# relife957/FastApriori

Hardware: AMD Instinct MI355X
Metric: itemsets/sec (mining wall-clock), T10I4D100M min_sup=0.001 (higher is better)
Workload: dtype int32/uint64-bitmap (exact integer counts); 1 GPU; model=T10I4D100M, global_batch=100000000, parallelism=dp1, n_itemsets=33139, min_count=100000

## Files before the change

### csrc/hip/regroup.hip

```cpp
#include "fa_hip.h"
#include "../host/fa_dl.h"
#include "../host/fa_regroup.h"

namespace fa {

constexpr int kRgThreads = 1024;
constexpr int kRgW = kRgThreads / 64;

struct RgLv {
  const int32_t* P;
  const int32_t* cnt;
  const int64_t* off;
  const int32_t* rows;
  char* scr;
  int64_t n, C, base;
  int64_t m;
};
struct RgArgs {
  RgLv lv[kDlMaxL];
  int32_t* perm;
  long long* stats;
};

__host__ __device__ inline int64_t rg_scratch_ints(int64_t n, int64_t C, int64_t m) {
  return ((C * (m + 5) + n) + 1) & ~(int64_t)1;
}
__host__ __device__ inline int64_t rg_scratch_bytes(int64_t n, int64_t C, int64_t m) {
  return (4 * rg_scratch_ints(n, C, m) + 8 * (n + 1) + 255) & ~(int64_t)255;
}

__device__ __forceinline__ int rg_find(const int32_t* __restrict__ P, int n, int m, const int32_t* __restrict__ s,
                                       int j) {
  int lo = 0, hi = n;
  while (lo < hi) {
    const int mid = (lo + hi) >> 1;
    const int r = cmp_skip(P + (int64_t)mid * m, s, m + 1, j);
    if (r == 0) return mid;
    if (r < 0) lo = mid + 1; else hi = mid;
  }
  return -1;
}

__global__ __launch_bounds__(kRgThreads) void k_dl_regroup(const RgArgs A) {
  extern __shared__ int rg_lds[];
  __shared__ int sh[2 * kRgW];
  __shared__ int fired;
  const RgLv& V = A.lv[blockIdx.x];
  const int tid = threadIdx.x;
  const int64_t C = V.C, base = V.base;
  if (V.n > kRgMaxRows) {
    for (int64_t c = tid; c < C; c += kRgThreads) A.perm[base + c] = (int32_t)(base + c);
    int pp = 0;
    for (int64_t i = tid; i < V.n; i += kRgThreads) pp += (V.cnt[i] + 7) >> 3;
    pp = wg_sum<kRgW>(pp, sh);
    if (tid == 0) {
      long long* s = A.stats + 4 * blockIdx.x;
      s[0] = s[1] = pp; s[2] = 0; s[3] = 1;
    }
    return;
  }
  const int n = (int)V.n, m = (int)V.m, k = m + 1;
  int32_t* const par = reinterpret_cast<int32_t*>(V.scr);
  int32_t* const asg = par + C * k;
  int32_t* const cho = asg + C;
  int32_t* const tmp = cho + C;
  int32_t* const cnt_out = tmp + C;
  int32_t* const ex_out = cnt_out + n;
  int64_t* const off_out = reinterpret_cast<int64_t*>(V.scr + 4 * rg_scratch_ints(n, C, m));
  int* u = rg_lds;
  int* u2 = rg_lds + n;
  int* const v = rg_lds + 2 * n;
  for (int i = tid; i < 3 * n; i += kRgThreads) rg_lds[i] = 0;
  if (tid == 0) fired = 0;
  __syncthreads();
  for (int64_t c = tid; c < C; c += kRgThreads) {
    const int32_t* s = V.rows + c * k;
    int lo = 0, hi = n;
    while (lo < hi) {
      const int mid = (lo + hi) >> 1;
      if (V.off[mid] <= c) lo = mid + 1; else hi = mid;
    }
    for (int j = 0; j < m; ++j) par[c * k + j] = rg_find(V.P, n, m, s, j);
    par[c * k + m] = lo - 1;
    asg[c] = -1;
    for (int j = 0; j < k; ++j) {
      const int p = par[c * k + j];
      if (p >= 0) atomicAdd(&u[p], 1);
    }
  }
  __syncthreads();
  int rounds = 0;
  for (int t = 0; t < kRgNThr; ++t) {
    const int thr = rg_thr(t);
    for (;;) {
      ++rounds;
      for (int64_t c = tid; c < C; c += kRgThreads) {
        if (asg[c] >= 0) continue;
        int best = -1, bp = -1;
        for (int j = k - 1; j >= 0; --j) {
          const int p = par[c * k + j];
          if (p < 0) continue;
          const int uu = u[p];
          if (uu >= thr && uu > best) { best = uu; bp = p; }
        }
        cho[c] = bp;
        if (bp >= 0) atomicAdd(&v[bp], 1);
      }
      __syncthreads();
      for (int64_t c = tid; c < C; c += kRgThreads) {
        if (asg[c] >= 0) continue;
        const int bp = cho[c];
        if (bp >= 0 && v[bp] >= thr) {
          asg[c] = bp;
          fired = 1;
          continue;
        }
        for (int j = 0; j < k; ++j) {
          const int p = par[c * k + j];
          if (p >= 0) atomicAdd(&u2[p], 1);
        }
      }
      __syncthreads();
      const int f = fired;
      __syncthreads();
      if (tid == 0) fired = 0;
      if (f) { int* x = u; u = u2; u2 = x; }
      for (int i = tid; i < n; i += kRgThreads) { u2[i] = 0; v[i] = 0; }
      __syncthreads();
      if (!f) break;
    }
  }
  for (int64_t c = tid; c < C; c += kRgThreads) atomicAdd(&v[asg[c]], 1);
  __syncthreads();
  int pc[2] = {0, 0}, tot[2];
  for (int i = tid; i < n; i += kRgThreads) {
    pc[0] += (v[i] + 7) >> 3;
    pc[1] += (V.cnt[i] + 7) >> 3;
  }
  wg_sum<kRgW>(pc, sh, tot);
  const bool keep = tot[0] >= tot[1];
  __syncthreads();
  if (keep) {
    for (int i = tid; i < n; i += kRgThreads) v[i] = 0;
    __syncthreads();
    for (int64_t c = tid; c < C; c += kRgThreads) {
      asg[c] = par[c * k + m];
      atomicAdd(&v[asg[c]], 1);
    }
    __syncthreads();
  }
  for (int i = tid; i < n; i += kRgThreads) cnt_out[i] = v[i];
  wg_scan_chunks<kRgW>(
      (int64_t)n, (int64_t)0, sh, [&](int64_t i) { return v[i]; },
      [&](int64_t i, int64_t before, int) { off_out[i] = before; });
  if (tid == 0) off_out[n] = C;
  for (int64_t c = tid; c < C; c += kRgThreads) {
    const int p = asg[c];
    tmp[off_out[p] + atomicAdd(&u2[p], 1)] = (int32_t)c;
  }
  __syncthreads();
  for (int64_t c = tid; c < C; c += kRgThreads) {
    const int p = asg[c];
    const int64_t o = off_out[p];
    const int a = v[p];
    int r = 0;
    for (int q = 0; q < a; ++q) r += tmp[o + q] < (int32_t)c ? 1 : 0;
    int j = m;
    if (!keep)
      for (j = k - 1; j > 0 && par[c * k + j] != p; --j) {}
    ex_out[o + r] = V.rows[c * k + j];
    A.perm[base + o + r] = (int32_t)(base + c);
  }
  if (tid == 0) {
    long long* s = A.stats + 4 * blockIdx.x;
    s[0] = tot[1]; s[1] = tot[0]; s[2] = rounds; s[3] = keep ? 1 : 0;
  }
}

__global__ __launch_bounds__(256) void k_dl_unpermute(const uint32_t* __restrict__ in, const int32_t* __restrict__ perm,
                                                      int64_t C, uint32_t* __restrict__ out) {
  const int64_t e = (int64_t)blockIdx.x * 256 + threadIdx.x;
  if (e < C) out[perm[e]] = in[e];
}

static inline int64_t rg_al(int64_t b) { return (b + 255) & ~(int64_t)255; }

static bool rg_eligible(const DlDesc* desc, int L) {
  if (L < 1 || L > kDlMaxL) return false;
  for (int l = 0; l < L; ++l)
    if (desc[l].m < 1 || desc[l].m > kDlInline || desc[l].n < 1 || desc[l].C < 1 || desc[l].C > INT32_MAX / 64)
      return false;
  return true;
}

}

using namespace fa;

FA_API int64_t fa_hip_dl_regroup_need(const DlDesc* desc, int L) {
  if (!rg_eligible(desc, L)) return 0;
  int64_t C = 0, b = 0;
  for (int l = 0; l < L; ++l) {
    C += desc[l].C;
    if (desc[l].n <= kRgMaxRows) b += rg_scratch_bytes(desc[l].n, desc[l].C, desc[l].m);
  }
  return rg_al(4 * C) + b;
}

FA_API int fa_hip_dl_regroup(const DlDesc* desc, int L, void* scratch, int64_t bytes, DlDesc* out, long long* stats,
                             hipStream_t st) {
  const int64_t need = fa_hip_dl_regroup_need(desc, L);
  if (need == 0 || scratch == nullptr || stats == nullptr || bytes < need) return 1;
  int64_t C = 0;
  for (int l = 0; l < L; ++l) C += desc[l].C;
  RgArgs A{};
  char* w = static_cast<char*>(scratch);
  A.perm = reinterpret_cast<int32_t*>(w);
  w += rg_al(4 * C);
  A.stats = stats;
  int64_t n_max = 1;
  for (int l = 0; l < L; ++l) {
    const DlDesc& d = desc[l];
    RgLv& V = A.lv[l];
    V.P = reinterpret_cast<const int32_t*>((intptr_t)d.P);
    V.cnt = reinterpret_cast<const int32_t*>((intptr_t)d.cnt);
    V.off = reinterpret_cast<const int64_t*>((intptr_t)d.off);
    V.rows = reinterpret_cast<const int32_t*>((intptr_t)d.rows);
    V.n = d.n; V.C = d.C; V.base = d.base; V.m = d.m;
    V.scr = w;
    out[l] = d;
    if (d.n > kRgMaxRows) continue;
    n_max = std::max(n_max, d.n);
    int32_t* cnt_out = reinterpret_cast<int32_t*>(w) + d.C * (d.m + 1) + 3 * d.C;
    out[l].cnt = (int64_t)(intptr_t)cnt_out;
    out[l].off = (int64_t)(intptr_t)(w + 4 * rg_scratch_ints(d.n, d.C, d.m));
    w += rg_scratch_bytes(d.n, d.C, d.m);
  }
  const size_t lds = 3 * sizeof(int) * (size_t)n_max;
  static bool lds_set = false;
  if (!lds_set) {
    const hipError_t e = hipFuncSetAttribute((const void*)k_dl_regroup, hipFuncAttributeMaxDynamicSharedMemorySize,
                                             (int)(3 * sizeof(int) * kRgMaxRows));
    if (e != hipSuccess) return (int)e;
    lds_set = true;
  }
  hipLaunchKernelGGL(k_dl_regroup, dim3((unsigned)L), dim3(kRgThreads), lds, st, A);
  FA_LAUNCH_RET();
}

FA_API int fa_hip_dl_unpermute(const uint32_t* in, const int32_t* perm, int64_t C, uint32_t* out, hipStream_t st) {
  if (C < 1) return 1;
  hipLaunchKernelGGL(k_dl_unpermute, dim3((unsigned)((C + 255) / 256)), dim3(256), 0, st, in, perm, C, out);
  FA_LAUNCH_RET();
}
```

### csrc/host/fa_regroup.h

```cpp
#pragma once
#include <stdint.h>

namespace fa {

constexpr int kRgNThr = 6;
constexpr int rg_thr(int t) { return t == 0 ? 8 : t == 1 ? 6 : t == 2 ? 4 : t == 3 ? 3 : t == 4 ? 2 : 1; }
constexpr int kRgMaxRows = 12288;
constexpr int kRgStats = 224;
static_assert(kRgStats + 4 * 32 <= 512, "the statistics end before the control block's bitset");

inline int rg_cmp_skip(const int32_t* a, const int32_t* s, int k, int p) {
  for (int i = 0, j = 0; i < k - 1; ++i, ++j) {
    if (j == p) ++j;
    const int32_t x = a[i], y = s[j];
    if (x != y) return x < y ? -1 : 1;
  }
  return 0;
}

}
```

### fastapriori_amd/ops/_native.py

```python
from __future__ import annotations

import ctypes as C
import os
import threading

from . import build as _build

_lock = threading.Lock()
_host = None
_hip = None

i32, i64, u64, dbl = C.c_int32, C.c_int64, C.c_uint64, C.c_double
vp, cp = C.c_void_p, C.c_char_p
I64P = C.POINTER(C.c_int64)
IP = C.POINTER(C.c_int)

_HOST_SIGS = {
    "fa_parse_file": (vp, [cp, i64, i64, C.c_int, C.c_int, IP]),
    "fa_parse_buffer": (vp, [cp, i64, C.c_int, C.c_int]),
    "fa_file_size": (i64, [cp]),
    "fa_next_line_start": (i64, [cp, i64, i64]),
    "fa_chunk_scan": (None, [vp, i64, vp]),
    "fa_txndb_info": (None, [vp, vp]),
    "fa_txndb_export": (None, [vp, vp, vp, vp, C.c_int]),
# ... 25 lines not shown
    "fa_slab_tail_cut": (C.c_int, [vp, C.c_int, i64, dbl, dbl]),
    "fa_trim_estimate": (None, [vp, i64, dbl, C.c_int, C.POINTER(dbl), C.POINTER(dbl)]),
    "fa_dl_layout": (cp, [C.c_int, I64P]),
    "fa_limits": (cp, [C.c_int, I64P]),
    "fa_query_limits": (cp, [C.c_int, I64P]),
    "fa_query_lds_bytes": (i64, [i64, i64, i64]),
    "fa_query_width": (C.c_int, [i64, i64, i64]),
    "fa_query_plan": (vp, [vp, vp, vp, i64, i64, i64, i64]),
    "fa_query_plan_info": (None, [vp, vp]),
    "fa_query_plan_export": (None, [vp, vp, vp, vp, vp, vp]),
    "fa_query_plan_free": (None, [vp]),
    "fa_query_count_cpu": (C.c_int, [vp, vp, i64, vp, i64, vp, i64, vp, vp, vp, vp, vp, i64, C.c_int]),
    "fa_f1_rank_numeric": (i64, [vp, i64, i64, vp, vp, vp]),
    "fa_rules_build": (vp, [vp, vp, vp, C.c_int, vp, C.c_int, vp]),
    "fa_rules_nante": (i64, [vp]),
    "fa_rules_nstats": (i64, [vp]),
    "fa_rules_export": (None, [vp, vp, vp, vp, vp, vp]),
    "fa_rules_free": (None, [vp]),
    "fa_rule_measures_cpu": (vp, [vp, vp, vp, vp, C.c_int, i64, dbl, C.c_int, dbl, C.c_int, i64, vp, C.c_int, vp]),
    "fa_rule_measures_nante": (i64, [vp]),
    "fa_rule_measures_export": (None, [vp] * 12),
    "fa_rule_measures_free": (None, [vp]),
    "fa_write_rules": (C.c_int, [cp, cp] + [vp] * 12 + [i64, C.c_int]),
    "fa_recommend_cpu": (None, [vp, vp, vp, i64, i32, vp, vp, i64, vp, C.c_int]),
    "fa_recommend_topn_cpu": (None, [vp, vp, vp, i64, i32, vp, vp, i64, i32, vp, C.c_int]),
    "fa_holdout_rank_cpu": (None, [vp, vp, vp, i64, i32, vp, vp, vp, i64, i32, vp, C.c_int]),
    "fa_recommend_combined_cpu": (None, [vp, vp, vp, vp, i64, i32, vp, vp, i64, i32, vp, vp, C.c_int]),
    "fa_holdout_rank_combined_cpu": (None, [vp, vp, vp, vp, i64, i32, vp, vp, vp, i64, i32, vp, C.c_int]),
    "fa_combine_wave_bytes": (i64, [i64]),
    "fa_combine_waves": (C.c_int, [i64]),
    "fa_combine_lds_max": (i64, []),
    "fa_condense_cpu": (C.c_int, [vp, vp, vp, vp, C.c_int, vp, vp, C.c_int]),
    "fa_write_freq_itemsets": (C.c_int, [cp, vp, vp, i32, vp, vp, vp, C.c_int, C.c_int, C.c_int]),
    "fa_cpu_histogram": (None, [vp, i64, i64, vp, C.c_int]),
    "fa_build_probe_table": (None, [vp, i64, C.c_int, C.c_uint32, vp, vp]),
    "fa_cpu_txn_freq_count": (None, [vp, vp, i64, vp, vp, C.c_int]),
    "fa_cpu_compress": (None, [vp, vp, vp, vp, i64, vp, vp, C.c_int]),
    "fa_cpu_build_bitmaps": (None, [vp, vp, vp, i64, i64, vp, C.c_int]),
    "fa_cpu_row_hash": (None, [vp, vp, i64, vp, vp, C.c_int]),
    "fa_cpu_pair_gram": (None, [vp, i32, i64, i64, vp, vp, C.c_int]),
    "fa_cpu_pair_horizontal": (None, [vp, vp, i64, vp, i32, vp, C.c_int]),
    "fa_cpu_count_candidates": (None, [vp, i64, i64, vp, i32, vp, vp, i64, vp, vp, C.c_int]),
}

_HIP_SIGS = {
    "fa_hip_histogram": (C.c_int, [vp, i64, i32, vp, vp]),
    "fa_hip_f1_rank": (C.c_int, [vp, i32, i64, C.c_int, vp, vp, vp]),
    "fa_hip_debug_la_qsum": (C.c_int, [vp, vp]),
    "fa_hip_win_alive": (C.c_int, [vp, i64, vp, C.c_int, i64, C.c_int, vp, vp, vp]),
    "fa_hip_win_compact": (C.c_int, [vp, i64, vp, C.c_int, i64, vp, vp, vp, i64, vp]),
    "fa_hip_debug_slab_max_wg": (None, [C.c_int]),
    "fa_hip_pairs_compact": (C.c_int, [vp, i64, i32, i64, vp, vp, vp, vp, vp, vp]),
    "fa_hip_f1_sketch": (C.c_int, [vp, i64, vp, vp, vp]),
    "fa_hip_f1_exact": (C.c_int, [vp, i64, vp, C.c_int, vp, vp]),
    "fa_hip_txn_freq_count": (C.c_int, [vp, vp, i64, i64, vp, vp, vp]),
    "fa_hip_compress_regs": (C.c_int, [C.c_int, vp, vp, vp, vp, i64, vp, vp, vp, vp, vp]),
    "fa_hip_ag_gen": (C.c_int, [vp, i64, C.c_int, C.c_int, vp, i64, vp, i64, vp, vp]),
    "fa_hip_ag_chain": (C.c_int, [vp, i64, C.c_int, C.c_int, vp, i64, vp, i64, C.c_int, dbl, i64, i64, vp, vp,
                                  C.c_int, dbl]),
    "fa_hip_ag_build": (C.c_int, [vp, i64, C.c_int, vp, C.c_uint32, C.c_int, vp, vp]),
    "fa_hip_ag_rows": (C.c_int, [vp, i64, C.c_int, vp, C.c_uint32, C.c_int, vp, vp, vp, vp, C.c_int, vp]),
    "fa_hip_cmp_agg": (C.c_int, [vp, vp, vp, i64, vp, vp, vp, C.c_int, vp]),
    "fa_hip_cmp_scan": (C.c_int, [vp, vp, i64, C.c_int, vp, vp, vp, vp, vp]),
    "fa_hip_cmp_emit": (C.c_int, [vp, vp, vp, i64, vp, vp, vp, vp, vp, vp, vp, vp, C.c_int, vp, vp, i64, vp, vp,
                                  vp]),
    "fa_hip_lr_rows": (C.c_int, [vp, vp, vp, i64, vp, C.c_int, vp, i64, vp]),
    "fa_hip_compress_regs_bc": (C.c_int, [vp, vp, vp, vp, i64, vp, vp, vp, vp, vp, i64, C.c_int, vp]),
    "fa_hip_block_counts_rows": (C.c_int, [vp, vp, vp, i64, vp, i64, C.c_int, vp, vp]),
    "fa_hip_block_bsum": (C.c_int, [vp, i64, i64, C.c_int, vp, vp]),
    "fa_hip_compress_staged": (C.c_int, [vp, vp, vp, i64, vp, vp, vp, vp, vp]),
    "fa_hip_compress_staged64": (C.c_int, [vp, vp, vp, i64, vp, vp, vp, vp, C.c_int, vp]),
    "fa_hip_count_slab_rec_cls": (C.c_int, [vp, vp, vp, i64, vp, C.c_int, C.c_int, vp, vp, C.c_int, C.c_int, vp,
                                            vp, C.c_int, C.c_int, vp, i64, vp, vp, vp, C.c_int]),
    "fa_hip_dl_level0": (C.c_int, [vp, vp, i64, i64, C.c_int, C.c_int, vp, i64, vp, vp, i64, dbl, dbl, vp, C.c_int,
                                   vp]),
    "fa_hip_dl_more": (C.c_int, [C.c_int, vp, i64, i64, vp, vp, dbl, C.c_int, dbl, dbl, i64, vp, vp, vp, vp]),
    "fa_hip_dl_plan": (C.c_int, [vp, C.c_int, vp, C.c_int, vp, vp, i64, vp, i64, vp, i64, C.c_int, vp]),
    "fa_hip_set_lane_deal": (None, [C.c_int]),
    "fa_hip_set_dl_tail": (None, [dbl, C.c_int]),
    "fa_hip_set_piece_part": (C.c_int, [C.c_int, C.c_int]),
    "fa_hip_set_dl_regroup": (None, [C.c_int]),
    "fa_hip_dl_regroup_last": (None, [vp]),
    "fa_hip_dl_regroup_need": (i64, [vp, C.c_int]),
    "fa_hip_dl_regroup": (C.c_int, [vp, C.c_int, vp, i64, vp, vp, vp]),
    "fa_hip_dl_unpermute": (C.c_int, [vp, vp, i64, vp, vp]),
    "fa_hip_dl_gpre_need": (i64, [vp, C.c_int]),
    "fa_hip_dl_plan_window": (C.c_int, [vp, C.c_int, vp, C.c_int, vp, vp, i64, vp, i64, vp, i64, i64, i64, C.c_int,
                                        vp]),
    "fa_hip_dl_plan_window_bits": (C.c_int, [vp, C.c_int, vp, C.c_int, vp, vp, vp, i64, vp, i64, vp, i64, i64, i64,
                                             C.c_int, vp]),
    "fa_hip_dl_chunk_bits": (C.c_int, [vp, C.c_int, C.c_int, vp, vp]),
    "fa_hip_dl_threshold": (C.c_int, [vp, C.c_int, vp, i64, vp, vp, vp, vp, vp, vp, i64, vp]),
    "fa_hip_trim_scan_count": (C.c_int, [vp, vp, i64, vp, C.c_int, C.c_int, vp, vp, vp, vp, vp]),
    "fa_hip_trim_emit": (C.c_int, [vp, vp, vp, C.c_int, i64, vp, vp, vp, vp, vp, vp, vp, vp]),
    "fa_hip_compress_wave": (C.c_int, [vp, vp, vp, vp, i64, vp, vp, vp, C.c_int, vp, vp]),
    "fa_hip_compress_lds": (C.c_int, [vp, vp, vp, vp, i64, vp, vp, vp, vp, vp, vp]),
    "fa_hip_dedup_probe": (C.c_int, [vp, vp, vp, i64, vp, vp, vp]),
    "fa_hip_row_hash": (C.c_int, [vp, vp, i64, vp, vp, vp]),
    "fa_hip_build_bitmaps": (C.c_int, [vp, vp, vp, i64, i32, i64, C.c_int, C.c_int, vp, vp, vp, C.c_int, vp]),
    "fa_hip_block_counts": (C.c_int, [vp, vp, i64, i32, vp, vp, C.c_int, vp]),
    "fa_hip_block_scatter": (C.c_int, [vp, vp, i64, i32, vp, vp, vp, C.c_int, vp]),
    "fa_hip_pair_queue16": (C.c_int, [vp, vp, vp, i64, C.c_int, i64, vp, vp, C.c_int, vp]),
    "fa_hip_pair_blocked": (C.c_int, [vp, vp, vp, i64, vp, i32, vp, i64, vp]),
    "fa_hip_pair_gram_mfma": (C.c_int, [vp, i32, i64, i64, C.c_int, i64, vp, C.c_int, C.c_uint32, C.c_int, vp]),
    "fa_hip_pair_gram_popc": (C.c_int, [vp, i32, i64, i64, C.c_int, i64, vp, vp, C.c_int, vp]),
    "fa_hip_count_candidates": (C.c_int, [vp, i64, i64, vp, C.c_int, vp, vp, vp, C.c_int, vp, vp, vp]),
    "fa_hip_recommend": (C.c_int, [vp, vp, vp, i64, i32, vp, vp, i64, vp, vp]),
    "fa_hip_recommend_indexed": (C.c_int, [vp, vp, vp, vp, vp, i64, i32, vp, vp, i64, vp, vp]),
    "fa_hip_recommend_topn": (C.c_int, [vp, vp, vp, i64, i32, vp, vp, i64, i32, vp, vp]),
    "fa_hip_recommend_topn_indexed": (C.c_int, [vp, vp, vp, vp, vp, i64, i32, vp, vp, i64, i32, vp, vp]),
    "fa_hip_holdout_rank": (C.c_int, [vp, vp, vp, i64, i32, vp, vp, vp, i64, i32, vp, vp]),
    "fa_hip_holdout_rank_indexed": (C.c_int, [vp, vp, vp, vp, vp, i64, i32, vp, vp, vp, i64, i32, vp, vp]),
    "fa_hip_recommend_combined": (C.c_int, [vp, vp, vp, vp, vp, vp, i64, i32, vp, vp, i64, i32, vp, vp, vp]),
    "fa_hip_holdout_rank_combined": (C.c_int, [vp, vp, vp, vp, vp, vp, i64, i32, vp, vp, vp, i64, i32, vp, vp]),
    "fa_hip_parse_tiles": (i64, [i64]),
    "fa_hip_tparse_tiles": (i64, [i64, i64]),
    "fa_hip_tline_count": (C.c_int, [vp, i64, i64, vp, vp]),
    "fa_hip_tparse": (C.c_int, [vp, i64, i64, i64, C.c_int, i64, vp, vp, vp, vp, vp, vp, vp, vp, vp]),
    "fa_hip_scan_small": (C.c_int, [C.c_int, vp, i64, vp, vp, vp]),
    "fa_hip_tcompact": (C.c_int, [vp, vp, i64, C.c_int, vp, vp, vp, vp, vp, vp, vp, i64, i64, vp, C.c_int, vp, vp, vp]),
    "fa_hip_hist_reduce": (C.c_int, [vp, C.c_int, vp, vp]),
    "fa_hip_line_count": (C.c_int, [vp, i64, vp, vp]),
    "fa_hip_line_ends": (C.c_int, [vp, i64, vp, vp, vp]),
    "fa_hip_parse_lines_dict": (C.c_int, [vp, vp, i64, vp, vp, vp, vp, vp, vp, vp, vp, vp, i64, vp]),
    "fa_hip_slot_remap": (C.c_int, [vp, i64, vp, vp]),
    "fa_hip_dict_verify": (C.c_int, [vp, vp, i64, vp, vp, vp, vp, i64, vp]),
    "fa_hip_compact_lines": (C.c_int, [vp, vp, vp, vp, vp, vp, vp, i64, vp, vp, vp]),
    "fa_hip_rule_gen": (C.c_int, [vp, i64, C.c_int, vp, i64, vp, vp, vp, vp, vp, vp]),
    "fa_hip_rule_cut": (C.c_int, [vp, vp, i64, C.c_int, vp, vp, vp, vp]),
    "fa_hip_rule_emit": (C.c_int, [vp, vp, vp, vp, vp, i64, vp, vp]),
    "fa_hip_rule_measures": (C.c_int, [vp, vp, vp, vp, vp, vp, C.c_int, i64, dbl, C.c_int, dbl, C.c_int, vp, vp, vp,
                                       vp, vp]),
    "fa_hip_rule_measures_emit": (C.c_int, [vp, vp, vp, vp, vp, vp, C.c_int, i64, C.c_int, vp, vp, i64, vp, vp, vp,
                                            vp, vp, vp, vp, vp, vp]),
    "fa_hip_rule_measures_fin": (C.c_int, [vp, vp, vp, i64, i64, vp, vp, vp, vp, vp, vp]),
    "fa_hip_sup_mark": (C.c_int, [vp, vp, vp, vp, vp, vp, C.c_int, vp, vp, vp, vp]),
    "fa_hip_query_count": (C.c_int, [vp, vp, i64, vp, i64, vp, vp, i64, vp, vp, vp, vp, vp, i64, C.c_int, vp]),
}


def _declare(lib, sigs):
    for name, (res, args) in sigs.items():
        fn = getattr(lib, name)
        fn.restype = res
        fn.argtypes = args
    return lib


BUILD_IDS: dict = {}


def _check_id(kind: str, lib, path: str) -> None:
    fn = lib.fa_build_id
    fn.restype, fn.argtypes = cp, []
    got = fn().decode("ascii", "replace")
    have_src = bool(_build.hip_sources() if kind == "hip" else _build.host_sources())
    want = _build.source_id(kind) if have_src else None
    BUILD_IDS[kind] = (got, want, path)
    override = kind == "hip" and bool(os.environ.get("FA_HIP_LIB"))
    if want is not None and got != want and not override:
        raise RuntimeError(f"{path} was built from other sources (build id {got}, these sources {want}): "
                           "rebuild with `python -m fastapriori_amd.ops.build`")


def host():
    global _host
# ... 33 lines not shown
```

### fastapriori_amd/ops/primitives.py

```python
from __future__ import annotations

import ctypes as C
import ctypes
import functools
import os
import time
from dataclasses import dataclass

import numpy as np
import torch

from ..tuning import TUNING
from ..utils.env import num_threads
from . import _native
from .host import rule_measures_plan, rules_gap_level, rules_not_closed

_I32, _I64 = torch.int32, torch.int64
PAIR_CHUNK_ROWS = 1 << 18


def _p(t: torch.Tensor | None) -> int | None:
    return None if t is None else t.data_ptr()


# ... 1745 lines not shown
        self.rows_hint = 0

    def grow(self, nbytes: int) -> None:
        self.ws = torch.empty(int(nbytes * 1.25) + (1 << 20), dtype=torch.uint8, device=self.dev)

    def post_buffers(self, F1: int, c_cap: int, rows_cap: int, gpre_n: int = 0):
        part_n = 8 * ((rows_cap + 255) // 256 + 2)
        b = self.post_bufs
        if (b is None or b["F1"] < F1 or b["c_cap"] < c_cap or b["part"].numel() < part_n
                or b["gpre"].numel() < gpre_n):
            F1, c_cap = max(F1, b["F1"] if b else 0), max(c_cap, b["c_cap"] if b else 0)
            part_n = max(part_n, b["part"].numel() if b else 0)
            gpre_n = max(gpre_n, b["gpre"].numel() if b else 1)
            b = self.post_bufs = dict(F1=F1, c_cap=c_cap,
                                      item_map=torch.empty(max(F1, 1), dtype=_I32, device=self.dev),
                                      rec=torch.empty(12 * c_cap + 12, dtype=_I32, device=self.dev),
                                      part=torch.empty(part_n, dtype=_I32, device=self.dev),
                                      out=torch.empty(c_cap, dtype=_I32, device=self.dev),
                                      gpre=torch.empty(max(gpre_n, 1), dtype=_I32, device=self.dev))
        return b


_DL_STATE: dict = {}


def device_level_state(dev) -> DeviceLevelState:
    st = _DL_STATE.get(dev)
    if st is None:
        st = _DL_STATE[dev] = DeviceLevelState(dev)
    return st


def dl_lds_budget(F1: int) -> int:
    return TUNING.slab_lds_bytes - slab_map_lds(F1)




def dl_bundle_gen(S: DeviceLevelState, P0: int, n_src: int | None, n_const: int, n_bound: int, m0: int, F1: int,
                  c_bound: int, lds: int, growth: float, max_levels: int, stream: int, post: bool = False,
                  accb: float = 4.0, tail_accb: float = 0.0, tail_levels: int = 0,
                  regroup: bool | None = None) -> np.ndarray:
    lib, K = _native.hip(), dl()
    info = np.zeros(2, dtype=np.int64)
    for _ in range(6):
        S.desc[:] = 0
        rc = lib.fa_hip_dl_level0(P0, n_src, n_const, n_bound, m0, F1, _p(S.ws), S.ws.numel(), _p(S.ctl),
                                  _p(S.ctl_h), c_bound, float(lds), float(accb), S.info.ctypes.data,
                                  int(max_levels <= 1), stream)
        if rc == 5:
            S.grow(int(S.info[0]))
            continue
        _native.check(rc, "fa_hip_dl_level0")
        d0 = S.desc[0]
        d0["P"], d0["cnt"], d0["off"], d0["rows"], d0["m"] = P0, S.info[1], S.info[2], S.info[3], m0
        if max_levels <= 1:
            c = S.ctl_h.numpy()
            d0["n"], d0["C"], d0["base"] = c[K.kDlNl], c[K.kDlCl], 0
            return c.copy()
        S.post.done = 0
        lane_deal(lib, S.rows_hint)
        lib.fa_hip_set_dl_tail(float(tail_accb) if post else 0.0, int(tail_levels))
        lib.fa_hip_set_dl_regroup(int(bool(TUNING.dl_regroup if regroup is None else regroup) and post))
        rc = lib.fa_hip_dl_more(F1, _p(S.ws), S.ws.numel(), int(S.info[0]), _p(S.ctl), _p(S.ctl_h), float(growth),
                                int(max_levels), float(lds), float(accb), int(c_bound), S.desc.ctypes.data,
                                info.ctypes.data,
                                stream, ctypes.addressof(S.post) if post else None)
        if rc == 5:
            S.grow(int(info[0]))
            continue
        _native.check(rc, "fa_hip_dl_more")
        return S.ctl_h.numpy().copy()
    raise RuntimeError("device bundle generation: workspace sizing did not converge")


def set_piece_part(part: int, nparts: int) -> None:
    _native.check(_native.hip().fa_hip_set_piece_part(int(part), int(nparts)), "fa_hip_set_piece_part")


def lane_deal(lib, rows: int) -> None:
    lib.fa_hip_set_lane_deal(int(0 <= TUNING.lane_deal_min_rows <= rows))


def dl_regroup(S: DeviceLevelState, L: int, dev) -> dict | None:
    lib = _native.hip()
    need = int(lib.fa_hip_dl_regroup_need(S.desc.ctypes.data, L))
    if need == 0:
        return None
    scratch = torch.empty(need, dtype=torch.uint8, device=dev)
    stats = torch.zeros((L, 4), dtype=_I64, device=dev)
    desc = S.desc.copy()
    st = torch.cuda.current_stream(dev).cuda_stream
    _native.check(lib.fa_hip_dl_regroup(S.desc.ctypes.data, L, _p(scratch), need, desc.ctypes.data, _p(stats), st),
                  "fa_hip_dl_regroup")
    C = int(S.desc["C"][:L].sum())
    perm = scratch[:4 * C].view(_I32)
    return dict(desc=desc, perm=perm, stats=stats, scratch=scratch)


def dl_regroup_last(S: DeviceLevelState | None = None) -> tuple[int, np.ndarray | None]:
    last = np.zeros(2, dtype=np.int64)
    _native.hip().fa_hip_dl_regroup_last(last.ctypes.data)
    S = S if S is not None else next(iter(_DL_STATE.values()), None)
    if last[0] == 0 or S is None:
        return int(last[0]), None
    at, L = int(_native.host().fa_dl_regroup_const(1)), int(last[1])
    return int(last[0]), S.ctl[at:at + 4 * L].cpu().numpy().reshape(L, 4)


def dl_unpermute(cnt: torch.Tensor, perm: torch.Tensor) -> torch.Tensor:
    out = torch.empty_like(cnt)
    st = torch.cuda.current_stream(cnt.device).cuda_stream
    _native.check(_native.hip().fa_hip_dl_unpermute(_p(cnt), _p(perm), cnt.numel(), _p(out), st),
                  "fa_hip_dl_unpermute")
    return out


def dl_plan(S: DeviceLevelState, L: int, F1: int, n_used: int, C: int, lds: int, dev, accb: float = 4.0,
            cnt_accb: float | None = None, pad: int = 0, desc=None) -> dict:
    st = torch.cuda.current_stream(dev).cuda_stream
    sw, cap = slab_width(n_used, C, lds, accb)
    if sw == 0 or C > cap:
        raise RuntimeError(f"device bundle of {C} candidates over {n_used} items does not fit one pass")
    if cnt_accb is not None and cnt_accb < accb:
        sw_c, cap_c, accb_c = ctypes.c_int(sw), ctypes.c_int64(cap), ctypes.c_double(accb)
        _native.host().fa_slab_acc_upgrade(int(n_used), int(C), float(lds), float(cnt_accb), ctypes.byref(sw_c),
                                           ctypes.byref(cap_c), ctypes.byref(accb_c))
        sw, cap, accb = int(sw_c.value), int(cap_c.value), float(accb_c.value)
    item_map = torch.empty(max(F1, 1), dtype=_I32, device=dev)
    rec = torch.empty(12 * C + 12, dtype=_I32, device=dev)
    desc = S.desc if desc is None else desc
    R = int(desc["n"][:L].sum())
    part = torch.empty(8 * max(1, (R + 255) // 256), dtype=_I32, device=dev)
    lib = _native.hip()
    gn = int(lib.fa_hip_dl_gpre_need(desc.ctypes.data, L))
    gpre = torch.empty(max(gn, 1), dtype=_I32, device=dev)
    lane_deal(lib, S.rows_hint)
    _native.check(lib.fa_hip_dl_plan(desc.ctypes.data, L, _p(S.ctl), F1, _p(item_map), _p(rec), C,
                                     _p(part), part.numel(), _p(gpre), gpre.numel(), slab_layout(sw, pad), st),
                  "fa_hip_dl_plan")
    out = torch.zeros(C, dtype=_I32, device=dev)
    return dict(sw=sw, pad=pad, cap=cap, item_map=item_map, rec=rec, out=out, n_used=n_used, C=C, gpre=gpre,
                accb=accb)


def dl_count_multipass(S: DeviceLevelState, F1: int, n_used: int, C: int, lds: int, roff, ranks, src, ncols: int,
                       wword, bm, bm_rows, sup_frac: float, dev, bmap=None, window_rows=None) -> torch.Tensor | None:
    acc16 = TUNING.dl_acc16 and wword is None
    accb = 2 if acc16 else 4
    sw, cap = slab_width(n_used, C, lds, accb)
    if sw == 0:
        return None
    st = _stream(ranks)
    lib = _native.hip()
    wins = None
    if TUNING.mp_window_items:
        wins = dl_window_plan(S, F1, C, lds, accb, st, dev)
    if not wins:
        cap = min(cap, C)
        cap = -(-C // -(-C // cap))
        wins = [(w0, min(C, w0 + cap), sw, None) for w0 in range(0, C, cap)]
    cap = max(w1 - w0 for w0, w1, _, _ in wins)
    item_map = torch.empty(max(F1, 1), dtype=_I32, device=dev)
    rec = torch.empty(12 * cap + 12, dtype=_I32, device=dev)
    R = int(S.desc[0]["n"])
    part = torch.empty(8 * max(1, (R + 255) // 256) + 16, dtype=_I32, device=dev)
    gn = int(lib.fa_hip_dl_gpre_need(S.desc.ctypes.data, 1))
    gpre = torch.empty(max(gn, 1), dtype=_I32, device=dev)
    out = torch.zeros(C, dtype=_I32, device=dev)
    npass, used_sum, rows_sum, trimmed = 0, 0, 0, 0
    lane_deal(lib, ncols)
    g_dev = _p(S.ctl) + 8 * dl().kDlPiecesI32
    for w0, w1, wsw, bits in wins:
        nu, rows_w, bits_p, bm_w, ncols_w = n_used, bm_rows, None, bm, ncols
        if bits is not None:
            used_w = np.flatnonzero(np.unpackbits(bits.view(np.uint8), bitorder="little")[:F1])
            nu = int(used_w.size)
# ... 140 lines not shown
```

Measured before the change: 922,600 itemsets/s.

## Split regroup into parallel parent lookup and LDS-resident compacted voting rounds

Result: faster. 937,600 itemsets/s (median of 6 runs) (+1.6%).

```diff
diff --git a/csrc/hip/regroup.hip b/csrc/hip/regroup.hip
--- a/csrc/hip/regroup.hip
+++ b/csrc/hip/regroup.hip
@@ -1,3 +1,6 @@
+#include <algorithm>
+#include <type_traits>
+
 #include "fa_hip.h"
 #include "../host/fa_dl.h"
 #include "../host/fa_regroup.h"
@@ -6,6 +9,8 @@
 
 constexpr int kRgThreads = 1024;
 constexpr int kRgW = kRgThreads / 64;
+constexpr int kRgPThreads = 256;
+constexpr uint16_t kRgNone = 0xFFFF;
 
 struct RgLv {
   const int32_t* P;
@@ -14,19 +19,26 @@
   const int32_t* rows;
   char* scr;
   int64_t n, C, base;
-  int64_t m;
+  int32_t m;
+  uint32_t blk0;
 };
 struct RgArgs {
   RgLv lv[kDlMaxL];
   int32_t* perm;
   long long* stats;
+  int64_t lds_cap;
+  long long* phase;
+  int32_t L;
 };
-
-__host__ __device__ inline int64_t rg_scratch_ints(int64_t n, int64_t C, int64_t m) {
-  return ((C * (m + 5) + n) + 1) & ~(int64_t)1;
+static_assert(sizeof(RgArgs) <= 4096, "kernel arguments");
+
+__host__ __device__ inline int64_t rg_off_at(int64_t n, int64_t C) { return (4 * (n + C) + 7) & ~(int64_t)7; }
+__host__ __device__ inline int64_t rg_par_at(int64_t n, int64_t C) { return rg_al16(rg_off_at(n, C) + 8 * (n + 1)); }
+__host__ __device__ inline int64_t rg_list_at(int64_t n, int64_t C, int64_t m) {
+  return rg_al16(rg_par_at(n, C) + 2 * C * (m + 1));
 }
 __host__ __device__ inline int64_t rg_scratch_bytes(int64_t n, int64_t C, int64_t m) {
-  return (4 * rg_scratch_ints(n, C, m) + 8 * (n + 1) + 255) & ~(int64_t)255;
+  return (rg_list_at(n, C, m) + 4 * ((C + 7) & ~(int64_t)7) + 255) & ~(int64_t)255;
 }
 
 __device__ __forceinline__ int rg_find(const int32_t* __restrict__ P, int n, int m, const int32_t* __restrict__ s,
@@ -41,15 +53,220 @@
   return -1;
 }
 
-__global__ __launch_bounds__(kRgThreads) void k_dl_regroup(const RgArgs A) {
-  extern __shared__ int rg_lds[];
+__global__ __launch_bounds__(kRgPThreads) void k_dl_rg_parents(const RgArgs A) {
+  int l = 0;
+  while (l + 1 < A.L && blockIdx.x >= A.lv[l + 1].blk0) ++l;
+  const RgLv& V = A.lv[l];
+  const int n = (int)V.n, m = V.m, C = (int)V.C;
+  if (V.n > kRgMaxRows) return;
+  const int64_t e = (int64_t)(blockIdx.x - V.blk0) * kRgPThreads + threadIdx.x;
+  if (e >= (int64_t)C * (m + 1)) return;
+  const int j = (int)((uint32_t)e / (uint32_t)C), c = (int)e - j * C;
+  int r;
+  if (j < m) {
+    r = rg_find(V.P, n, m, V.rows + (int64_t)c * (m + 1), j);
+  } else {
+    int lo = 0, hi = n;
+    while (lo < hi) {
+      const int mid = (lo + hi) >> 1;
+      if (V.off[mid] <= c) lo = mid + 1; else hi = mid;
+    }
+    r = lo - 1;
+  }
+  reinterpret_cast<uint16_t*>(V.scr + rg_par_at(n, C))[e] = r < 0 ? kRgNone : (uint16_t)r;
+}
+
+__device__ __forceinline__ void pk_inc(uint32_t* a, int p) { atomicAdd(&a[p >> 1], 1u << (16 * (p & 1))); }
+__device__ __forceinline__ int pk_get(const uint32_t* a, int p) {
+  return (int)reinterpret_cast<const uint16_t*>(a)[p];
+}
+
+constexpr int kRgMaxK = kDlInline + 1;
+template <int K>
+__device__ __forceinline__ int rg_vote(const uint16_t* par, const uint32_t* u, int C, int thr, int c, int (&ps)[K]) {
+#pragma unroll
+  for (int j = 0; j < K; ++j) ps[j] = (int)par[j * C + c];
+  int us[K];
+#pragma unroll
+  for (int j = 0; j < K; ++j) us[j] = ps[j] != kRgNone ? pk_get(u, ps[j]) : -1;
+  int best = -1, bp = -1;
+#pragma unroll
+  for (int j = K - 1; j >= 0; --j)
+    if (us[j] >= thr && us[j] > best) { best = us[j]; bp = ps[j]; }
+  return bp;
+}
+
+__device__ __forceinline__ void rg_load8(const uint16_t* p, int (&it)[8]) {
+  const uint4 q = *reinterpret_cast<const uint4*>(p);
+  const uint32_t w[4] = {q.x, q.y, q.z, q.w};
+#pragma unroll
+  for (int h = 0; h < 8; ++h) it[h] = (int)((w[h >> 1] >> (16 * (h & 1))) & 0xFFFFu);
+}
+__device__ __forceinline__ void rg_load8(const int32_t* p, int (&it)[8]) {
+  const int4 a = reinterpret_cast<const int4*>(p)[0], b = reinterpret_cast<const int4*>(p)[1];
+  it[0] = a.x; it[1] = a.y; it[2] = a.z; it[3] = a.w;
+  it[4] = b.x; it[5] = b.y; it[6] = b.z; it[7] = b.w;
+}
+
+template <bool kLds, int K>
+__device__ __forceinline__ void rg_level(const RgArgs& A, const RgLv& V, uint32_t* lds, int* sh, int* fired) {
+  using Li = typename std::conditional<kLds, uint16_t, int32_t>::type;
+  const int tid = threadIdx.x;
+  constexpr int k = K, m = K - 1;
+  const int n = (int)V.n, C = (int)V.C, nh = (n + 1) >> 1;
+  const int64_t base = V.base;
+  int32_t* const cnt_out = reinterpret_cast<int32_t*>(V.scr);
+  int32_t* const ex_out = cnt_out + n;
+  int64_t* const off_out = reinterpret_cast<int64_t*>(V.scr + rg_off_at(n, C));
+  uint16_t* const gpar = reinterpret_cast<uint16_t*>(V.scr + rg_par_at(n, C));
+  uint32_t* u = lds;
+  uint32_t* u2 = lds + nh;
+  uint32_t* const v = lds + 2 * nh;
+  char* const lists = reinterpret_cast<char*>(lds) + rg_lds_counters(n);
+  uint16_t* const par = kLds ? reinterpret_cast<uint16_t*>(lists) : gpar;
+  Li* const list = kLds ? reinterpret_cast<Li*>(lists + rg_lds_par(C, m))
+                        : reinterpret_cast<Li*>(V.scr + rg_list_at(n, C, m));
+  auto mark = [&](int i) {
+    if (A.phase != nullptr && tid == 0) A.phase[4 * blockIdx.x + i] = (long long)wall_clock64();
+  };
+  mark(0);
+  for (int i = tid; i < 3 * nh; i += kRgThreads) lds[i] = 0;
+  __syncthreads();
+  const int E = k * C, nv = E >> 3;
+  for (int i = tid; i < nv; i += kRgThreads) {
+    const uint4 q = reinterpret_cast<const uint4*>(gpar)[i];
+    if (kLds) reinterpret_cast<uint4*>(par)[i] = q;
+    const uint32_t w[4] = {q.x, q.y, q.z, q.w};
+#pragma unroll
+    for (int h = 0; h < 8; ++h) {
+      const int p = (int)((w[h >> 1] >> (16 * (h & 1))) & 0xFFFFu);
+      if (p != kRgNone) pk_inc(u, p);
+    }
+  }
+  for (int e = 8 * nv + tid; e < E; e += kRgThreads) {
+    const uint16_t p = gpar[e];
+    if (kLds) par[e] = p;
+    if (p != kRgNone) pk_inc(u, p);
+  }
+  for (int c = tid; c < C; c += kRgThreads) list[c] = (Li)c;
+  __syncthreads();
+  mark(1);
+  constexpr int kDead = kLds ? 0xFFFF : -1;
+  int left = C, rounds = 0;
+  for (int t = 0; t < kRgNThr; ++t) {
+    const int thr = rg_thr(t);
+    for (;;) {
+      ++rounds;
+#pragma unroll 2
+      for (int i = tid; i < left; i += kRgThreads) {
+        int ps[K];
+        const int bp = rg_vote<K>(par, u, C, thr, (int)list[i], ps);
+        if (bp >= 0) pk_inc(v, bp);
+      }
+      __syncthreads();
+#pragma unroll 2
+      for (int i = tid; i < left; i += kRgThreads) {
+        const int c = (int)list[i];
+        int ps[K];
+        const int bp = rg_vote<K>(par, u, C, thr, c, ps);
+        if (bp >= 0 && pk_get(v, bp) >= thr) {
+          par[c] = (uint16_t)bp;
+          list[i] = (Li)kDead;
+          *fired = 1;
+          continue;
+        }
+#pragma unroll
+        for (int j = 0; j < K; ++j)
+          if (ps[j] != kRgNone) pk_inc(u2, ps[j]);
+      }
+      __syncthreads();
+      const bool f = *fired != 0;
+      if (f) {
+      int it[8];
+      left = (int)wg_scan_chunks<kRgW>(
+          (int64_t)((left + 7) >> 3), (int64_t)0, sh,
+          [&](int64_t g) {
+            rg_load8(list + 8 * g, it);
+            int kept = 0;
+#pragma unroll
+            for (int h = 0; h < 8; ++h) {
+              if (8 * (int)g + h >= left) it[h] = kDead;
+              kept += it[h] != kDead ? 1 : 0;
+            }
+            return kept;
+          },
+          [&](int64_t, int64_t before, int) {
+            int r = (int)before;
+#pragma unroll
+            for (int h = 0; h < 8; ++h)
+              if (it[h] != kDead) list[r++] = (Li)it[h];
+          });
+      if (tid == 0) *fired = 0;
+      uint32_t* x = u; u = u2; u2 = x;
+      }
+      for (int i = tid; i < nh; i += kRgThreads) { u2[i] = 0; v[i] = 0; }
+      __syncthreads();
+      if (!f) break;
+    }
+  }
+  mark(2);
+  for (int c = tid; c < C; c += kRgThreads) pk_inc(v, par[c]);
+  __syncthreads();
+  int pc[2] = {0, 0}, tot[2];
+  for (int i = tid; i < n; i += kRgThreads) {
+    pc[0] += (pk_get(v, i) + 7) >> 3;
+    pc[1] += (V.cnt[i] + 7) >> 3;
+  }
+  wg_sum<kRgW>(pc, sh, tot);
+  const bool keep = tot[0] >= tot[1];
+  __syncthreads();
+  if (keep) {
+    for (int i = tid; i < nh; i += kRgThreads) v[i] = 0;
+    __syncthreads();
+    for (int c = tid; c < C; c += kRgThreads) {
+      const uint16_t p = par[m * C + c];
+      par[c] = p;
+      pk_inc(v, p);
+    }
+    __syncthreads();
+  }
+  int32_t* const cur = reinterpret_cast<int32_t*>(lds);
+  wg_scan_chunks<kRgW>(
+      (int64_t)n, (int64_t)0, sh, [&](int64_t i) { return pk_get(v, (int)i); },
+      [&](int64_t i, int64_t before, int a) {
+        cnt_out[i] = a;
+        off_out[i] = before;
+        cur[i] = (int32_t)before;
+      });
+  if (tid == 0) off_out[n] = C;
+  for (int c = tid; c < C; c += kRgThreads) list[atomicAdd(&cur[par[c]], 1)] = (Li)c;
+  __syncthreads();
+  for (int c = tid; c < C; c += kRgThreads) {
+    const int p = par[c];
+    const int a = pk_get(v, p), o = cur[p] - a;
+    int r = 0;
+    for (int q = 0; q < a; ++q) r += (int)list[o + q] < c ? 1 : 0;
+    int j = m;
+    if (!keep)
+      for (j = k - 1; j > 0 && par[j * C + c] != p; --j) {}
+    ex_out[o + r] = V.rows[(int64_t)c * k + j];
+    A.perm[base + o + r] = (int32_t)(base + c);
+  }
+  if (tid == 0) {
+    long long* s = A.stats + 4 * blockIdx.x;
+    s[0] = tot[1]; s[1] = tot[0]; s[2] = rounds; s[3] = keep ? 1 : 0;
+  }
+  mark(3);
+}
+
+__global__ __launch_bounds__(kRgThreads) void k_dl_rg_rounds(const RgArgs A) {
+  extern __shared__ __attribute__((aligned(16))) uint32_t rg_lds[];
   __shared__ int sh[2 * kRgW];
   __shared__ int fired;
   const RgLv& V = A.lv[blockIdx.x];
   const int tid = threadIdx.x;
-  const int64_t C = V.C, base = V.base;
   if (V.n > kRgMaxRows) {
-    for (int64_t c = tid; c < C; c += kRgThreads) A.perm[base + c] = (int32_t)(base + c);
+    for (int64_t c = tid; c < V.C; c += kRgThreads) A.perm[V.base + c] = (int32_t)(V.base + c);
     int pp = 0;
     for (int64_t i = tid; i < V.n; i += kRgThreads) pp += (V.cnt[i] + 7) >> 3;
     pp = wg_sum<kRgW>(pp, sh);
@@ -59,122 +276,19 @@
     }
     return;
   }
-  const int n = (int)V.n, m = (int)V.m, k = m + 1;
-  int32_t* const par = reinterpret_cast<int32_t*>(V.scr);
-  int32_t* const asg = par + C * k;
-  int32_t* const cho = asg + C;
-  int32_t* const tmp = cho + C;
-  int32_t* const cnt_out = tmp + C;
-  int32_t* const ex_out = cnt_out + n;
-  int64_t* const off_out = reinterpret_cast<int64_t*>(V.scr + 4 * rg_scratch_ints(n, C, m));
-  int* u = rg_lds;
-  int* u2 = rg_lds + n;
-  int* const v = rg_lds + 2 * n;
-  for (int i = tid; i < 3 * n; i += kRgThreads) rg_lds[i] = 0;
   if (tid == 0) fired = 0;
-  __syncthreads();
-  for (int64_t c = tid; c < C; c += kRgThreads) {
-    const int32_t* s = V.rows + c * k;
-    int lo = 0, hi = n;
-    while (lo < hi) {
-      const int mid = (lo + hi) >> 1;
-      if (V.off[mid] <= c) lo = mid + 1; else hi = mid;
-    }
-    for (int j = 0; j < m; ++j) par[c * k + j] = rg_find(V.P, n, m, s, j);
-    par[c * k + m] = lo - 1;
-    asg[c] = -1;
-    for (int j = 0; j < k; ++j) {
-      const int p = par[c * k + j];
-      if (p >= 0) atomicAdd(&u[p], 1);
-    }
-  }
-  __syncthreads();
-  int rounds = 0;
-  for (int t = 0; t < kRgNThr; ++t) {
-    const int thr = rg_thr(t);
-    for (;;) {
-      ++rounds;
-      for (int64_t c = tid; c < C; c += kRgThreads) {
-        if (asg[c] >= 0) continue;
-        int best = -1, bp = -1;
-        for (int j = k - 1; j >= 0; --j) {
-          const int p = par[c * k + j];
-          if (p < 0) continue;
-          const int uu = u[p];
-          if (uu >= thr && uu > best) { best = uu; bp = p; }
-        }
-        cho[c] = bp;
-        if (bp >= 0) atomicAdd(&v[bp], 1);
-      }
-      __syncthreads();
-      for (int64_t c = tid; c < C; c += kRgThreads) {
-        if (asg[c] >= 0) continue;
-        const int bp = cho[c];
-        if (bp >= 0 && v[bp] >= thr) {
-          asg[c] = bp;
-          fired = 1;
-          continue;
-        }
-        for (int j = 0; j < k; ++j) {
-          const int p = par[c * k + j];
-          if (p >= 0) atomicAdd(&u2[p], 1);
-        }
-      }
-      __syncthreads();
-      const int f = fired;
-      __syncthreads();
-      if (tid == 0) fired = 0;
-      if (f) { int* x = u; u = u2; u2 = x; }
-      for (int i = tid; i < n; i += kRgThreads) { u2[i] = 0; v[i] = 0; }
-      __syncthreads();
-      if (!f) break;
-    }
-  }
-  for (int64_t c = tid; c < C; c += kRgThreads) atomicAdd(&v[asg[c]], 1);
-  __syncthreads();
-  int pc[2] = {0, 0}, tot[2];
-  for (int i = tid; i < n; i += kRgThreads) {
-    pc[0] += (v[i] + 7) >> 3;
-    pc[1] += (V.cnt[i] + 7) >> 3;
-  }
-  wg_sum<kRgW>(pc, sh, tot);
-  const bool keep = tot[0] >= tot[1];
-  __syncthreads();
-  if (keep) {
-    for (int i = tid; i < n; i += kRgThreads) v[i] = 0;
-    __syncthreads();
-    for (int64_t c = tid; c < C; c += kRgThreads) {
-      asg[c] = par[c * k + m];
-      atomicAdd(&v[asg[c]], 1);
-    }
-    __syncthreads();
-  }
-  for (int i = tid; i < n; i += kRgThreads) cnt_out[i] = v[i];
-  wg_scan_chunks<kRgW>(
-      (int64_t)n, (int64_t)0, sh, [&](int64_t i) { return v[i]; },
-      [&](int64_t i, int64_t before, int) { off_out[i] = before; });
-  if (tid == 0) off_out[n] = C;
-  for (int64_t c = tid; c < C; c += kRgThreads) {
-    const int p = asg[c];
-    tmp[off_out[p] + atomicAdd(&u2[p], 1)] = (int32_t)c;
-  }
-  __syncthreads();
-  for (int64_t c = tid; c < C; c += kRgThreads) {
-    const int p = asg[c];
-    const int64_t o = off_out[p];
-    const int a = v[p];
-    int r = 0;
-    for (int q = 0; q < a; ++q) r += tmp[o + q] < (int32_t)c ? 1 : 0;
-    int j = m;
-    if (!keep)
-      for (j = k - 1; j > 0 && par[c * k + j] != p; --j) {}
-    ex_out[o + r] = V.rows[c * k + j];
-    A.perm[base + o + r] = (int32_t)(base + c);
-  }
-  if (tid == 0) {
-    long long* s = A.stats + 4 * blockIdx.x;
-    s[0] = tot[1]; s[1] = tot[0]; s[2] = rounds; s[3] = keep ? 1 : 0;
-  }
+  const bool fits = rg_lds_fits(V.n, V.C, V.m, A.lds_cap);
+#define FA_RG_K(K)                                         \
+  case K:                                                  \
+    if (fits) rg_level<true, K>(A, V, rg_lds, sh, &fired); \
+    else rg_level<false, K>(A, V, rg_lds, sh, &fired);     \
+    break;
+  static_assert(kRgMaxK == 13, "one case per k = m + 1 (rg_eligible: 1 <= m <= kDlInline)");
+  switch (V.m + 1) {
+    FA_RG_K(2) FA_RG_K(3) FA_RG_K(4) FA_RG_K(5) FA_RG_K(6) FA_RG_K(7)
+    FA_RG_K(8) FA_RG_K(9) FA_RG_K(10) FA_RG_K(11) FA_RG_K(12) FA_RG_K(13)
+  }
+#undef FA_RG_K
 }
 
 __global__ __launch_bounds__(256) void k_dl_unpermute(const uint32_t* __restrict__ in, const int32_t* __restrict__ perm,
@@ -193,9 +307,22 @@
   return true;
 }
 
+static int64_t g_rg_lds_cap = kRgLdsMax;
+static long long* g_rg_phase = nullptr;
+
 }
 
 using namespace fa;
+
+FA_API void fa_hip_set_dl_regroup_lds(int64_t bytes) {
+  g_rg_lds_cap = bytes < 0 ? kRgLdsMax : std::min<int64_t>(bytes, kRgLdsMax);
+}
+
+FA_API void fa_hip_debug_dl_regroup_phases(long long* buf) { g_rg_phase = buf; }
+
+FA_API int64_t fa_hip_dl_regroup_lds(int64_t n, int64_t C, int64_t m) {
+  return rg_lds_fits(n, C, m, INT64_MAX) ? rg_lds_all(n, C, m) : -1;
+}
 
 FA_API int64_t fa_hip_dl_regroup_need(const DlDesc* desc, int L) {
   if (!rg_eligible(desc, L)) return 0;
@@ -211,6 +338,7 @@
                              hipStream_t st) {
   const int64_t need = fa_hip_dl_regroup_need(desc, L);
   if (need == 0 || scratch == nullptr || stats == nullptr || bytes < need) return 1;
+  if ((intptr_t)scratch & 15) return 1;
   int64_t C = 0;
   for (int l = 0; l < L; ++l) C += desc[l].C;
   RgArgs A{};
@@ -218,7 +346,10 @@
   A.perm = reinterpret_cast<int32_t*>(w);
   w += rg_al(4 * C);
   A.stats = stats;
-  int64_t n_max = 1;
+  A.lds_cap = g_rg_lds_cap;
+  A.phase = g_rg_phase;
+  A.L = L;
+  int64_t lds = 16, blocks = 0;
   for (int l = 0; l < L; ++l) {
     const DlDesc& d = desc[l];
     RgLv& V = A.lv[l];
@@ -226,25 +357,30 @@
     V.cnt = reinterpret_cast<const int32_t*>((intptr_t)d.cnt);
     V.off = reinterpret_cast<const int64_t*>((intptr_t)d.off);
     V.rows = reinterpret_cast<const int32_t*>((intptr_t)d.rows);
-    V.n = d.n; V.C = d.C; V.base = d.base; V.m = d.m;
+    V.n = d.n; V.C = d.C; V.base = d.base; V.m = (int32_t)d.m;
     V.scr = w;
+    V.blk0 = (uint32_t)blocks;
     out[l] = d;
     if (d.n > kRgMaxRows) continue;
-    n_max = std::max(n_max, d.n);
-    int32_t* cnt_out = reinterpret_cast<int32_t*>(w) + d.C * (d.m + 1) + 3 * d.C;
-    out[l].cnt = (int64_t)(intptr_t)cnt_out;
-    out[l].off = (int64_t)(intptr_t)(w + 4 * rg_scratch_ints(d.n, d.C, d.m));
+    lds = std::max(lds, rg_lds_bytes(d.n, d.C, d.m, A.lds_cap));
+    blocks += (d.C * (d.m + 1) + kRgPThreads - 1) / kRgPThreads;
+    out[l].cnt = (int64_t)(intptr_t)w;
+    out[l].off = (int64_t)(intptr_t)(w + rg_off_at(d.n, d.C));
     w += rg_scratch_bytes(d.n, d.C, d.m);
   }
-  const size_t lds = 3 * sizeof(int) * (size_t)n_max;
   static bool lds_set = false;
   if (!lds_set) {
-    const hipError_t e = hipFuncSetAttribute((const void*)k_dl_regroup, hipFuncAttributeMaxDynamicSharedMemorySize,
-                                             (int)(3 * sizeof(int) * kRgMaxRows));
+    const hipError_t e =
+        hipFuncSetAttribute((const void*)k_dl_rg_rounds, hipFuncAttributeMaxDynamicSharedMemorySize, (int)kRgLdsMax);
     if (e != hipSuccess) return (int)e;
     lds_set = true;
   }
-  hipLaunchKernelGGL(k_dl_regroup, dim3((unsigned)L), dim3(kRgThreads), lds, st, A);
+  if (blocks > 0) {
+    hipLaunchKernelGGL(k_dl_rg_parents, dim3((unsigned)blocks), dim3(kRgPThreads), 0, st, A);
+    const hipError_t e = hipGetLastError();
+    if (e != hipSuccess) return (int)e;
+  }
+  hipLaunchKernelGGL(k_dl_rg_rounds, dim3((unsigned)L), dim3(kRgThreads), (size_t)lds, st, A);
   FA_LAUNCH_RET();
 }
 
diff --git a/csrc/host/fa_regroup.h b/csrc/host/fa_regroup.h
--- a/csrc/host/fa_regroup.h
+++ b/csrc/host/fa_regroup.h
@@ -6,6 +6,21 @@
 constexpr int kRgNThr = 6;
 constexpr int rg_thr(int t) { return t == 0 ? 8 : t == 1 ? 6 : t == 2 ? 4 : t == 3 ? 3 : t == 4 ? 2 : 1; }
 constexpr int kRgMaxRows = 12288;
+
+constexpr int64_t kRgLdsMax = 160 * 1024 - 512;
+constexpr int64_t rg_al16(int64_t b) { return (b + 15) & ~(int64_t)15; }
+constexpr int64_t rg_lds_counters(int64_t n) { return rg_al16(3 * 4 * ((n + 1) / 2)); }
+constexpr int64_t rg_lds_par(int64_t C, int64_t m) { return rg_al16(2 * C * (m + 1)); }
+constexpr int64_t rg_lds_all(int64_t n, int64_t C, int64_t m) {
+  return rg_lds_counters(n) + rg_lds_par(C, m) + rg_al16(2 * C);
+}
+constexpr bool rg_lds_fits(int64_t n, int64_t C, int64_t m, int64_t cap) {
+  return C < 0xFFFF && rg_lds_all(n, C, m) <= cap;
+}
+constexpr int64_t rg_lds_bytes(int64_t n, int64_t C, int64_t m, int64_t cap) {
+  return rg_lds_fits(n, C, m, cap) ? rg_lds_all(n, C, m) : rg_lds_counters(n);
+}
+static_assert(rg_lds_counters(kRgMaxRows) <= kRgLdsMax, "the counters of any level fit");
 constexpr int kRgStats = 224;
 static_assert(kRgStats + 4 * 32 <= 512, "the statistics end before the control block's bitset");
 
diff --git a/fastapriori_amd/ops/_native.py b/fastapriori_amd/ops/_native.py
--- a/fastapriori_amd/ops/_native.py
+++ b/fastapriori_amd/ops/_native.py
@@ -131,6 +131,9 @@
     "fa_hip_set_dl_regroup": (None, [C.c_int]),
     "fa_hip_dl_regroup_last": (None, [vp]),
     "fa_hip_dl_regroup_need": (i64, [vp, C.c_int]),
+    "fa_hip_set_dl_regroup_lds": (None, [i64]),
+    "fa_hip_dl_regroup_lds": (i64, [i64, i64, i64]),
+    "fa_hip_debug_dl_regroup_phases": (None, [vp]),
     "fa_hip_dl_regroup": (C.c_int, [vp, C.c_int, vp, i64, vp, vp, vp]),
     "fa_hip_dl_unpermute": (C.c_int, [vp, vp, i64, vp, vp]),
     "fa_hip_dl_gpre_need": (i64, [vp, C.c_int]),
diff --git a/fastapriori_amd/ops/primitives.py b/fastapriori_amd/ops/primitives.py
--- a/fastapriori_amd/ops/primitives.py
+++ b/fastapriori_amd/ops/primitives.py
@@ -1851,7 +1851,7 @@
     lib.fa_hip_set_lane_deal(int(0 <= TUNING.lane_deal_min_rows <= rows))
 
 
-def dl_regroup(S: DeviceLevelState, L: int, dev) -> dict | None:
+def dl_regroup(S: DeviceLevelState, L: int, dev, lds_cap: int | None = None) -> dict | None:
     lib = _native.hip()
     need = int(lib.fa_hip_dl_regroup_need(S.desc.ctypes.data, L))
     if need == 0:
@@ -1860,8 +1860,14 @@
     stats = torch.zeros((L, 4), dtype=_I64, device=dev)
     desc = S.desc.copy()
     st = torch.cuda.current_stream(dev).cuda_stream
-    _native.check(lib.fa_hip_dl_regroup(S.desc.ctypes.data, L, _p(scratch), need, desc.ctypes.data, _p(stats), st),
-                  "fa_hip_dl_regroup")
+    if lds_cap is not None:
+        lib.fa_hip_set_dl_regroup_lds(int(lds_cap))
+    try:
+        rc = lib.fa_hip_dl_regroup(S.desc.ctypes.data, L, _p(scratch), need, desc.ctypes.data, _p(stats), st)
+    finally:
+        if lds_cap is not None:
+            lib.fa_hip_set_dl_regroup_lds(-1)
+    _native.check(rc, "fa_hip_dl_regroup")
     C = int(S.desc["C"][:L].sum())
     perm = scratch[:4 * C].view(_I32)
     return dict(desc=desc, perm=perm, stats=stats, scratch=scratch)
```
